# MaxWolf-01/sentinel2-landcover-classification

Measured on AMD Instinct MI355X. Metric: Sentinel-2 256x256x13 tiles/sec fwd+bwd, higher is better.
Workload: dtype f32

## Files before the change

### include/s2k_ops.h

```cpp
#ifndef S2K_OPS_H
#define S2K_OPS_H

#define S2K_N_T 12
#define S2K_N_N 4
#define S2K_N_D 24
#define S2K_N_F 6

#define S2K_BASE_WS 0
#define S2K_BASE_PARAMS 1
#define S2K_BASE_GRADS 2
#define S2K_BASE_BUFS 3
#define S2K_BASE_X 4
#define S2K_BASE_OUT 5
#define S2K_BASE_DOUT 6
#define S2K_BASE_NOISE 7
#define S2K_BASE_WGS 8
#define S2K_BASE_CONST 9
#define S2K_BASE_Y 10
#define S2K_BASE_AUX 11
#define S2K_BASE_WPACK 12
#define S2K_BASE_DX 13
#define S2K_N_BASES 14

#define S2K_PRO_NONE 0
#define S2K_PRO_AFFINE 1
#define S2K_PRO_SILU 2
#define S2K_PRO_RELU 3
#define S2K_PRO_GELU 4
#define S2K_MODE_CONV 0
#define S2K_MODE_CONVT_SCATTER 1
#define S2K_MODE_GATHER2X2 2
#define S2K_FLAG_SIDE 1
#define S2K_FLAG_JOIN 2
#define S2K_FLAG_BF16 4
#define S2K_FLAG_Q4 16
#define S2K_FLAG_DMA 8
#define S2K_FLAG_RES_GELU_GRAD 32
#define S2K_FLAG_SPLIT 64
#define S2K_FLAG_CHAIN 128

#define S2K_OP_MEMSET 1
#define S2K_MEMSET_T_DST 0
#define S2K_MEMSET_N_BYTES 0

#define S2K_OP_AXPY 2
#define S2K_AXPY_T_X 0
#define S2K_AXPY_T_Y 1
#define S2K_AXPY_N_COUNT 0

#define S2K_OP_WEIGHT_PACK 3
#define S2K_WEIGHT_PACK_T_TABLE 0
#define S2K_WEIGHT_PACK_T_SRC 1
#define S2K_WEIGHT_PACK_T_DST 2
#define S2K_WEIGHT_PACK_N_TOTAL 0
#define S2K_WEIGHT_PACK_N_BF16_BASE 1
#define S2K_WEIGHT_PACK_N_Q4_BASE 2
#define S2K_WEIGHT_PACK_N_SPLIT_BASE 3
#define S2K_WEIGHT_PACK_D_N_ENTRIES 0

#define S2K_OP_CONV 4
#define S2K_CONV_T_X1 0
#define S2K_CONV_T_BNV1 1
#define S2K_CONV_T_GATE1 2
#define S2K_CONV_T_X2 3
#define S2K_CONV_T_BNV2 4
#define S2K_CONV_T_WT 5
#define S2K_CONV_T_BIAS 6
#define S2K_CONV_T_Y 7
#define S2K_CONV_T_STATS 8
#define S2K_CONV_T_RES 9
#define S2K_CONV_T_SCRATCH 10
#define S2K_CONV_T_WTB 11
// ... 722 lines not shown
```

### sentinel2-landcover-classification_amd/csrc/dwconv.hip

```cpp
#include <stdlib.h>

#include <algorithm>

#include "common.h"

namespace s2k {

struct DwP {
    const float* x;
    const float* bnv;
    const float* w;
    const float* dy;
    float* out;
    double* stats;
    int B, C, H, W, K, S, PT, PL, HO, WO, pro, beta, nrep;
    int PPB, RT, bands, IRt, LW;
    int XG, LPP, lwp_shift;
    int vps_shift;
    float inv_xg;
    int bloop, cgroups;
    BnFold fold;
};

__device__ __forceinline__ int chan_of(int64_t plane, int C) { return (int)((uint32_t)plane % (uint32_t)C); }
// ... 358 lines not shown
        }
        __builtin_amdgcn_wave_barrier();
#pragma unroll
        for (int g = 0; g < NG; ++g) {
            const int gi = li + 64 * g, r = gi / XGW, xg = gi % XGW;
            float o[4] = {0.f, 0.f, 0.f, 0.f};
            const float* t0 = t + r * TW + 4 * xg;
#pragma unroll
            for (int ky = 0; ky < K; ++ky) {
                float win[12];
                read_window<3>(t0 + ky * TW, win);
#pragma unroll
                for (int kx = 0; kx < K; ++kx)
#pragma unroll
                    for (int j = 0; j < 4; ++j) o[j] = fmaf(wk[ky * K + kx], win[4 - PADK + j + kx], o[j]);
            }
            if (ok) {
                *reinterpret_cast<f32x4*>(p.out + off + 4 * li + 256 * g) = f32x4{o[0], o[1], o[2], o[3]};
#pragma unroll
                for (int j = 0; j < 4; ++j) { s += o[j]; q = fmaf(o[j], o[j], q); }
            }
        }
#pragma unroll
        for (int g = 0; g < NG; ++g) cur[g] = nxt[g];
        hcur = hnxt;
    }
    if (p.stats) {
        const double sd = wave_sum_d((double)s), qd = wave_sum_d((double)q);
        if (lane == 0) {
            double* st = p.stats + (int64_t)((blockIdx.x + blockIdx.y) % p.nrep) * 2 * p.C;
            atomic_add_d(st + c, sd);
            atomic_add_d(st + p.C + c, qd);
        }
    }
}

template <int K, int PRO, int W, int R = W>
__global__ void __launch_bounds__(NTHREADS) dwconv_wgrad_plane_kernel(const DwP p, int bchunk) {
    constexpr int PADK = (K - 1) / 2;
    constexpr bool BAND = R != W;
    constexpr int NB = W / R, GPP = R * W / 4, NG = GPP > 64 ? GPP / 64 : 1, LPP = GPP > 64 ? 64 : GPP, PW = 64 / LPP, XGW = W / 4;
    constexpr int HG = BAND ? (K - 1) * XGW : 0;
    constexpr int TH = R + K - 1, TW = W + 8, TILE = TH * TW, HW = W * W;
    static_assert(HG <= 64 && (!BAND || PW == 1) && W % R == 0, "band geometry");
    extern __shared__ __attribute__((aligned(16))) float smem[];
    const int lane = threadIdx.x & 63, wave = threadIdx.x >> 6;
    const int c = blockIdx.x * 4 + wave;
    if (c >= p.C) return;
    const int n_items = p.B * NB;
    const int i_lo = blockIdx.y * bchunk, i_hi = min(n_items, i_lo + bchunk);
    float sc = 1.0f, sh = 0.0f;
    if (PRO != S2K_PRO_NONE) { sc = p.bnv[c]; sh = p.bnv[p.C + c]; }
    float* tiles = smem + wave * (2 * PW * TILE);
    for (int i = lane; i < 2 * PW * TILE; i += 64) tiles[i] = 0.0f;
    const int sub = lane / LPP, li = lane % LPP;
    const int64_t bstride = (int64_t)p.C * HW, coff = (int64_t)c * HW;
    const f32x4 zero = {0.f, 0.f, 0.f, 0.f};
    const int hrow = lane / XGW, hxg = lane % XGW;
    const int h_trow = hrow < PADK ? hrow : R + hrow;
    const int h_dy = hrow < PADK ? hrow - PADK : R + hrow - PADK;
    auto item_off = [&](int it, int& y0) -> int64_t {
        const int b = BAND ? it / NB : it;
        y0 = BAND ? (it - b * NB) * R : 0;
        return (int64_t)b * bstride + coff + (int64_t)y0 * W;
    };
    f32x4 cur[NG], dcur[NG], hcur = zero;
// ... 1242 lines not shown
    p.dbeta1 = ref_ptr<float>(c, a1.t[S2K_BN_BWD_APPLY_T_DBETA]);
    p.x = ref_ptr<const float>(c, dg.t[S2K_DWCONV_DGRAD_T_XRAW]);
    p.bnv2 = ref_ptr<const float>(c, dg.t[S2K_DWCONV_DGRAD_T_BNV]);
    p.w = ref_ptr<const float>(c, dg.t[S2K_DWCONV_DGRAD_T_WT]);
    p.dw = ref_ptr<float>(c, wg.t[S2K_DWCONV_WGRAD_T_DW]);
    p.g = ref_ptr<float>(c, dg.t[S2K_DWCONV_DGRAD_T_G]);
    p.gamma2 = ref_ptr<const float>(c, a2.t[S2K_BN_BWD_APPLY_T_GAMMA]);
    p.dgamma2 = ref_ptr<float>(c, a2.t[S2K_BN_BWD_APPLY_T_DGAMMA]);
    p.dbeta2 = ref_ptr<float>(c, a2.t[S2K_BN_BWD_APPLY_T_DBETA]);
    const void* all[] = {p.d, p.dy, p.ydw, p.bnv1, p.mulbc, p.addbc, p.ps, p.gamma1, p.dgamma1, p.dbeta1, p.x, p.bnv2, p.w, p.dw, p.g, p.gamma2,
                         p.dgamma2, p.dbeta2};
    for (const void* q : all) {
        if (bad(q)) { set_error("dw_bwd_chain: null base"); return S2K_EFAULT; }
        if (!q) { set_error("dw_bwd_chain: missing tensor"); return S2K_EINVAL; }
    }
    p.B = dg.d[0]; p.C = dg.d[1];
    const int W = dg.d[3], K = dg.d[4];
    p.inv_count1 = 1.0 / (double)a1.n[S2K_BN_BWD_APPLY_N_COUNT];
    p.inv_count2 = 1.0 / (double)a2.n[S2K_BN_BWD_APPLY_N_COUNT];
    p.addscale = a1.f[S2K_BN_BWD_APPLY_F_ADDSCALE];
    const int pw = W == 8 ? 4 : 1;
    const size_t lds = ((size_t)4 * 2 * 2 * pw * (W + K - 1) * (W + 8) + 16 + 4 * K * K) * sizeof(float);
    if (lds > 64 * 1024) { set_error("dw_bwd_chain: tile too large (%zu B)", lds); return S2K_EINVAL; }
    const dim3 grid(p.C);
    if (K == 3 && W == 8) hipLaunchKernelGGL((dw_bwd_chain_kernel<3, 8>), grid, dim3(NTHREADS), lds, c.stream, p);
    else if (K == 3 && W == 16) hipLaunchKernelGGL((dw_bwd_chain_kernel<3, 16>), grid, dim3(NTHREADS), lds, c.stream, p);
    else if (K == 5 && W == 8) hipLaunchKernelGGL((dw_bwd_chain_kernel<5, 8>), grid, dim3(NTHREADS), lds, c.stream, p);
    else if (K == 5 && W == 16) hipLaunchKernelGGL((dw_bwd_chain_kernel<5, 16>), grid, dim3(NTHREADS), lds, c.stream, p);
    else { set_error("dw_bwd_chain: unsupported plane %d, k %d", W, K); return S2K_EINVAL; }
    g_s2k_variant = 10;
    return S2K_OK;
}

}
```

### sentinel2-landcover-classification_amd/csrc/s2k_api.hip

```cpp
#include <cstdarg>
#include <cstdio>
#include <cstring>
#include <mutex>
#include <vector>

#include <stdlib.h>

#include "common.h"

namespace s2k {

static thread_local char g_err[512] = "";
thread_local int g_s2k_variant = 0;

void set_error(const char* fmt, ...) {
    va_list ap;
    va_start(ap, fmt);
    vsnprintf(g_err, sizeof(g_err), fmt, ap);
    va_end(ap);
}

int launch_conv(const S2kOp&, const Ctx&);
int launch_wgrad(const S2kOp&, const Ctx&);
int launch_dwconv_fwd(const S2kOp&, const Ctx&);
// ... 19 lines not shown
int launch_chan_ln_bwd(const S2kOp&, const Ctx&);
int launch_act_bwd(const S2kOp&, const Ctx&);
int launch_act_fwd(const S2kOp&, const Ctx&);
int launch_attn_fwd(const S2kOp&, const Ctx&);
int launch_attn_bwd(const S2kOp&, const Ctx&);
int launch_mae_mask_index(const S2kOp&, const Ctx&);
int launch_token_gather(const S2kOp&, const Ctx&);
int launch_token_scatter(const S2kOp&, const Ctx&);
int launch_patchify(const S2kOp&, const Ctx&);
int launch_mae_loss_fwd(const S2kOp&, const Ctx&);
int launch_mae_loss_bwd(const S2kOp&, const Ctx&);
int launch_transpose_cl(const S2kOp&, const Ctx&);
int launch_drop_gate(const S2kOp&, const Ctx&);
int launch_confusion(const S2kOp&, const Ctx&);
int launch_tile_prep(const S2kOp&, const Ctx&);
int launch_se_bn_sums(const S2kOp&, const Ctx&);
int launch_se_bn_combine(const S2kOp&, const Ctx&);
int launch_space_to_depth(const S2kOp&, const Ctx&);
int launch_se_fc_wgrad(const S2kOp&, const Ctx&);
int launch_ids_to_dec_idx(const S2kOp&, const Ctx&);
int launch_upsample_zero(const S2kOp&, const Ctx&);
int launch_im2col(const S2kOp&, const Ctx&);
int launch_tile_label_hist(const S2kOp&, const Ctx&);
int launch_tile_moments(const S2kOp&, const Ctx&);
int launch_window_blend(const S2kOp&, const Ctx&);
int launch_seg_stats(const S2kOp&, const Ctx&);
int launch_seg_hist(const S2kOp&, const Ctx&);
int launch_grad_clip(const S2kOp&, const Ctx&);
int launch_tile_radix_hist(const S2kOp&, const Ctx&);
int launch_tile_rank_pick(const S2kOp&, const Ctx&);
int launch_tile_quicklook(const S2kOp&, const Ctx&);
int launch_class_overlay(const S2kOp&, const Ctx&);
int launch_dw_bwd_chain(const S2kOp*, const Ctx&);
int launch_adam(float*, const float*, float*, float*, int64_t, double, double, double, double, double, int, hipStream_t);
int launch_mfma_selftest(const float*, const float*, float*, hipStream_t);
int check_mae_panels(const float*, const float*, const float*, const float*, const double*, unsigned char*, float*, int, int, int, int,
                     int, int, int, const int*, int, const int*, int, int, int);
int launch_mae_panels(const float*, const float*, const float*, const float*, const double*, unsigned char*, float*, int, int, int, int,
                      int, int, int, const int*, int, const int*, int, int, int, hipStream_t);
int check_classmap_filter(const void*, int, const int*, void*, int, int, int, int, int, int, int, unsigned, unsigned, int, const unsigned char*,
                          const int*, const int*, int, unsigned long long*, unsigned long long*);
int launch_classmap_filter(const void*, int, const int*, void*, int, int, int, int, int, int, int, unsigned, unsigned, int, const unsigned char*,
                           const int*, const int*, int, unsigned long long*, unsigned long long*, hipStream_t);
int check_classmap_components(const void*, int, const int*, int, int, int, int, int, unsigned, int*, int*, unsigned long long*, unsigned*);
int launch_classmap_components(const void*, int, const int*, int, int, int, int, int, unsigned, int*, int*, unsigned long long*, unsigned*,
                               hipStream_t);
int check_classmap_sieve(const void*, int, const int*, void*, int, int, int, int, int, int, unsigned, int, const int*, const int*,
                         unsigned long long*, const unsigned char*, const int*, const int*, int, unsigned long long*, unsigned long long*,
                         unsigned*);
int launch_classmap_sieve(const void*, int, const int*, void*, int, int, int, int, int, int, unsigned, int, const int*, const int*,
                          unsigned long long*, const unsigned char*, const int*, const int*, int, unsigned long long*, unsigned long long*,
                          unsigned*, hipStream_t);
int check_classmap_distance(const void*, int, const int*, int, int, int, int, int, unsigned, int, unsigned, void*, int*, int*, const void*, int,
                            const int*, int, unsigned long long*);
int launch_classmap_distance(const void*, int, const int*, int, int, int, int, int, unsigned, int, unsigned, void*, int*, int*, const void*, int,
                             const int*, int, unsigned long long*, hipStream_t);
size_t classmap_distance_workspace(int, int, int);
int check_calibration(const float*, int, const void*, int, const int*, int, int, int, unsigned, const float*, int, int, int, float, int, float*,
                      void*, int, unsigned long long*, unsigned long long*, unsigned long long*);
int launch_calibration(const float*, int, const void*, int, const int*, int, int, int, unsigned, const float*, int, int, int, float, int, float*,
                       void*, int, unsigned long long*, unsigned long long*, unsigned long long*, hipStream_t);
int check_rasterize(const int*, int, const int*, const int*, int, const int*, int, const int*, int, int, int, void*, int, int, int, int, void*,
                    long long*, int*);
int launch_rasterize(const int*, int, const int*, const int*, int, const int*, int, const int*, int, int, int, void*, int, int, int, int, void*,
                     long long*, int*, hipStream_t);
size_t rasterize_workspace(int, int);
// ... 172 lines not shown
};

static int try_dw_chain(const S2kOp* ops, int i, int end, const Ctx& c, int* rc) {
    if (!(ops[i].flags & S2K_FLAG_CHAIN) || i + 3 >= end) return 0;
    const S2kOp &a1 = ops[i], &wg = ops[i + 1], &dg = ops[i + 2], &a2 = ops[i + 3];
    if (a1.kind != S2K_OP_BN_BWD_APPLY || wg.kind != S2K_OP_DWCONV_WGRAD || dg.kind != S2K_OP_DWCONV_DGRAD || a2.kind != S2K_OP_BN_BWD_APPLY) return 0;
    if ((a1.flags | wg.flags | dg.flags | a2.flags) & (S2K_FLAG_BF16 | S2K_FLAG_SPLIT)) return 0;
    const int64_t dy = a1.t[S2K_BN_BWD_APPLY_T_DY], x = dg.t[S2K_DWCONV_DGRAD_T_XRAW], g = dg.t[S2K_DWCONV_DGRAD_T_G];
    if (dy < 0 || a1.t[S2K_BN_BWD_APPLY_T_GP] != dy || a1.t[S2K_BN_BWD_APPLY_T_COEF] >= 0 || a1.t[S2K_BN_BWD_APPLY_T_PS] < 0 ||
        a1.t[S2K_BN_BWD_APPLY_T_MULBC] < 0 || a1.t[S2K_BN_BWD_APPLY_T_ADDBC] < 0 || a1.d[S2K_BN_BWD_APPLY_D_ACT] != S2K_PRO_SILU ||
        a1.d[S2K_BN_BWD_APPLY_D_EVAL] || a1.d[S2K_BN_BWD_APPLY_D_OUT_BF16] || a1.n[S2K_BN_BWD_APPLY_N_COUNT] <= 0) return 0;
    if (wg.t[S2K_DWCONV_WGRAD_T_DY] != dy || dg.t[S2K_DWCONV_DGRAD_T_DY] != dy || x < 0 || wg.t[S2K_DWCONV_WGRAD_T_X] != x ||
        dg.t[S2K_DWCONV_DGRAD_T_BNV] < 0 || wg.t[S2K_DWCONV_WGRAD_T_BNV] != dg.t[S2K_DWCONV_DGRAD_T_BNV] || g < 0 || g == dy || g == x ||
        dg.t[S2K_DWCONV_DGRAD_T_STATS2] < 0) return 0;
    for (int k = 0; k <= 10; ++k)
        if (wg.d[k] != dg.d[k]) return 0;
    const int B = dg.d[0], C = dg.d[1], H = dg.d[2], W = dg.d[3], K = dg.d[4];
    if (B <= 0 || C <= 0 || H != W || (W != 8 && W != 16) || (K != 3 && K != 5) || dg.d[5] != 1 || dg.d[6] != (K - 1) / 2 || dg.d[7] != (K - 1) / 2 ||
        dg.d[8] != H || dg.d[9] != W || dg.d[10] != S2K_PRO_SILU || dg.d[S2K_DWCONV_DGRAD_D_BETA] != 0) return 0;
    if ((int64_t)B * C * H * W * 4 >= 0x7ffffff0ll) return 0;
    if (a2.t[S2K_BN_BWD_APPLY_T_GP] != g || a2.t[S2K_BN_BWD_APPLY_T_DY] != g || a2.t[S2K_BN_BWD_APPLY_T_Y] != x ||
        a2.t[S2K_BN_BWD_APPLY_T_BNV] != dg.t[S2K_DWCONV_DGRAD_T_BNV] || a2.t[S2K_BN_BWD_APPLY_T_STATS2] != dg.t[S2K_DWCONV_DGRAD_T_STATS2] ||
        a2.t[S2K_BN_BWD_APPLY_T_COEF] >= 0 || a2.t[S2K_BN_BWD_APPLY_T_PS] >= 0 || a2.t[S2K_BN_BWD_APPLY_T_MULBC] >= 0 ||
        a2.t[S2K_BN_BWD_APPLY_T_ADDBC] >= 0 || a2.d[S2K_BN_BWD_APPLY_D_ACT] != S2K_PRO_NONE || a2.d[S2K_BN_BWD_APPLY_D_EVAL] ||
        a2.d[S2K_BN_BWD_APPLY_D_OUT_BF16] || a2.n[S2K_BN_BWD_APPLY_N_COUNT] <= 0) return 0;
    const int HW = H * W;
    if (a1.d[S2K_BN_BWD_APPLY_D_B] != B || a1.d[S2K_BN_BWD_APPLY_D_C] != C || a1.d[S2K_BN_BWD_APPLY_D_HW] != HW ||
        a2.d[S2K_BN_BWD_APPLY_D_B] != B || a2.d[S2K_BN_BWD_APPLY_D_C] != C || a2.d[S2K_BN_BWD_APPLY_D_HW] != HW) return 0;
    g_s2k_variant = 0;
    *rc = check_launch(launch_dw_bwd_chain(&ops[i], c), ops[i], i);
    return 4;
}

int s2k_program_run(const S2kOp* ops, int begin, int end, void* const* bases, int n_bases, void* stream) {
    if (!ops || !bases || begin < 0 || end < begin) { set_error("program_run: bad arguments"); return S2K_EINVAL; }
    hipStream_t main_st = static_cast<hipStream_t>(stream);
    DeviceGuard guard(main_st);
    Ctx c{bases, n_bases, main_st};
    bool any_side = false;
    for (int i = begin; i < end && !any_side; ++i) any_side = (ops[i].flags & S2K_FLAG_SIDE) != 0;
    SideQueue* sq = any_side ? lease_side_queue(guard.dev) : nullptr;
    bool side_busy = false;
    bool main_dirty = true;
    auto join = [&]() {
        if (!side_busy) return;
        (void)hipEventRecord(sq->join, sq->stream);
        (void)hipStreamWaitEvent(main_st, sq->join, 0);
        side_busy = false;
    };
    int rc = S2K_OK;
    for (int i = begin; i < end; ++i) {
        const S2kOp& op = ops[i];
        if ((op.flags & S2K_FLAG_CHAIN) && i + 3 < end) {
            if ((op.flags | ops[i + 1].flags | ops[i + 2].flags | ops[i + 3].flags) & S2K_FLAG_JOIN) join();
            const int used = try_dw_chain(ops, i, end, c, &rc);
            if (used) {
                main_dirty = true;
                if (rc != S2K_OK) break;
                i += used - 1;
                continue;
            }
        }
        if ((op.flags & S2K_FLAG_SIDE) && sq) {
            if (main_dirty) {
                (void)hipEventRecord(sq->fork, main_st);
                (void)hipStreamWaitEvent(sq->stream, sq->fork, 0);
                main_dirty = false;
            }
            Ctx cs{bases, n_bases, sq->stream};
            rc = check_launch(dispatch(op, cs), op, i);
            side_busy = true;
        } else {
            if (op.flags & S2K_FLAG_JOIN) join();
            rc = check_launch(dispatch(op, c), op, i);
            main_dirty = true;
        }
        if (rc != S2K_OK) break;
    }
    join();
    release_side_queue(guard.dev, sq);
    return rc;
}

int s2k_op_launch(const S2kOp* op, void* const* bases, int n_bases, void* stream) {
    if (!op || !bases) { set_error("op_launch: bad arguments"); return S2K_EINVAL; }
    DeviceGuard guard(static_cast<hipStream_t>(stream));
    Ctx c{bases, n_bases, static_cast<hipStream_t>(stream)};
    return check_launch(dispatch(*op, c), *op, 0);
}

static int profile_impl(const S2kOp* ops, int begin, int end, void* const* bases, int n_bases, void* stream, float* ms_by_kind,
                        int* launches_by_kind, float* ms_per_op, int* variant_per_op);

int s2k_program_profile(const S2kOp* ops, int begin, int end, void* const* bases, int n_bases, void* stream, float* ms_by_kind,
                        int* launches_by_kind) {
// ... 3 lines not shown
int s2k_program_profile_ops(const S2kOp* ops, int begin, int end, void* const* bases, int n_bases, void* stream,
                            float* ms_per_op) {
    float ms[S2K_N_KINDS + 1];
    int cnt[S2K_N_KINDS + 1];
    return profile_impl(ops, begin, end, bases, n_bases, stream, ms, cnt, ms_per_op, nullptr);
}

int s2k_program_profile_variants(const S2kOp* ops, int begin, int end, void* const* bases, int n_bases, void* stream,
                                 float* ms_per_op, int* variant_per_op) {
    float ms[S2K_N_KINDS + 1];
    int cnt[S2K_N_KINDS + 1];
    if (!ms_per_op || !variant_per_op) { set_error("program_profile_variants: bad arguments"); return S2K_EINVAL; }
    return profile_impl(ops, begin, end, bases, n_bases, stream, ms, cnt, ms_per_op, variant_per_op);
}

static int profile_impl(const S2kOp* ops, int begin, int end, void* const* bases, int n_bases, void* stream, float* ms_by_kind,
                        int* launches_by_kind, float* ms_per_op, int* variant_per_op) {
    if (!ops || !bases || !ms_by_kind || !launches_by_kind || begin < 0 || end < begin) {
        set_error("program_profile: bad arguments");
        return S2K_EINVAL;
    }
    hipStream_t st = static_cast<hipStream_t>(stream);
    DeviceGuard guard(st);
    Ctx c{bases, n_bases, st};
    const int n = end - begin;
    hipEvent_t* ev = new hipEvent_t[n + 1];
    for (int i = 0; i <= n; ++i) hipEventCreate(&ev[i]);
    int rc = S2K_OK;
    hipEventRecord(ev[0], st);
    int done = 0;
    std::vector<char> fused(n, 0);
    for (int i = 0; i < n; ++i) {
        g_s2k_variant = 0;
        const int used = try_dw_chain(ops, begin + i, end, c, &rc);
        if (!used) rc = check_launch(dispatch(ops[begin + i], c), ops[begin + i], begin + i);
        if (rc != S2K_OK) break;
        for (int k = 0; k < (used ? used : 1); ++k) {
            if (variant_per_op) variant_per_op[i + k] = g_s2k_variant;
            hipEventRecord(ev[i + k + 1], st);
            if (k) fused[i + k] = 1;
        }
        if (used) i += used - 1;
        done = i + 1;
    }
    hipStreamSynchronize(st);
    if (rc == S2K_OK) {
        for (int k = 0; k <= S2K_N_KINDS; ++k) { ms_by_kind[k] = 0.0f; launches_by_kind[k] = 0; }
        for (int i = 0; i < done; ++i) {
            float ms = 0.0f;
            if (!fused[i]) hipEventElapsedTime(&ms, ev[i], ev[i + 1]);
            const int k = ops[begin + i].kind;
            if (ms_per_op) ms_per_op[i] = ms;
            if (k > 0 && k <= S2K_N_KINDS && !fused[i]) { ms_by_kind[k] += ms; launches_by_kind[k] += 1; }
        }
    }
    for (int i = 0; i <= n; ++i) hipEventDestroy(ev[i]);
    delete[] ev;
    return rc;
}

int s2k_adam_step(float* p, const float* g, float* m, float* v, int64_t n, double lr, double beta1, double beta2, double eps,
                  double weight_decay, int step, void* stream) {
    DeviceGuard guard(static_cast<hipStream_t>(stream));
    const int rc = launch_adam(p, g, m, v, n, lr, beta1, beta2, eps, weight_decay, step, static_cast<hipStream_t>(stream));
    if (rc != S2K_OK) return rc;
    const hipError_t e = hipGetLastError();
    if (e != hipSuccess) { set_error("adam: %s", hipGetErrorString(e)); return S2K_EHIP; }
// ... 123 lines not shown
```

### sentinel2-landcover-classification_amd/plan/opdefs.py

```python
from __future__ import annotations

N_T, N_N, N_D, N_F = 12, 4, 24, 6
OP_BYTES = 8 + 8 * N_T + 8 * N_N + 4 * N_D + 4 * N_F
assert OP_BYTES == 256

BASES = ["WS", "PARAMS", "GRADS", "BUFS", "X", "OUT", "DOUT", "NOISE", "WGS", "CONST", "Y", "AUX", "WPACK", "DX"]
BASE = {n: i for i, n in enumerate(BASES)}

def stats_replicas(C: int) -> int:
    return max(1, min(64, 4096 // max(C, 1)))


PRO_NONE, PRO_AFFINE, PRO_SILU, PRO_RELU, PRO_GELU = 0, 1, 2, 3, 4
ACT_NONE, ACT_SILU, ACT_RELU, ACT_GELU = 0, 2, 3, 4
ACT_MUL = 5
MODE_CONV, MODE_CONVT_SCATTER, MODE_GATHER2X2 = 0, 1, 2
FLAG_SIDE, FLAG_JOIN = 1, 2
FLAG_BF16 = 4
FLAG_Q4 = 16
FLAG_RES_GELU_GRAD = 32
FLAG_SPLIT = 64
FLAG_DMA = 8
FLAG_CHAIN = 128

FOLD_T, FOLD_N, FOLD_D, FOLD_F = ["FSTATS", "FGAMMA", "FBETA", "FRM", "FRV"], ["FCOUNT"], ["FNREP"], ["FEPS", "FMOM"]
FOLD_KINDS = ("DWCONV_FWD", "SE_POOL", "BN_RESIDUAL")

OPS: dict[str, tuple[list[str], list[str], list[str], list[str]]] = {
    "MEMSET": (["DST"], ["BYTES"], [], []),
    "AXPY": (["X", "Y"], ["COUNT"], [], []),
    "WEIGHT_PACK": (["TABLE", "SRC", "DST"], ["TOTAL", "BF16_BASE", "Q4_BASE", "SPLIT_BASE"], ["N_ENTRIES"], []),
    "CONV": (["X1", "BNV1", "GATE1", "X2", "BNV2", "WT", "BIAS", "Y", "STATS", "RES", "SCRATCH", "WTB"], [],
             ["B", "C1", "C2", "H", "W", "M", "KH", "KW", "STRIDE", "PAD_T", "PAD_L", "HO", "WO",
              "PRO1", "PRO2", "MODE", "W_SM", "W_SK", "W_ST", "FLIP", "BETA", "YC", "NREP", "X1_BF16"], []),
    "WGRAD": (["P", "BNVP", "GATEP", "Q", "BNVQ", "GATEQ", "WGS"], [],
              ["B", "M", "C", "CTOT", "H", "W", "KH", "KW", "STRIDE", "PAD_T", "PAD_L", "HO", "WO",
               "PROP", "PROQ", "MODE", "P_BF16"], []),
    "WGRAD_FINALIZE": (["TABLE", "WGS", "GRADS"], ["TOTAL"], ["N_ENTRIES"], []),
    "DWCONV_FWD": (["X", "BNV", "WT", "Y", "STATS"] + FOLD_T, FOLD_N,
                   ["B", "C", "H", "W", "K", "STRIDE", "PAD_T", "PAD_L", "HO", "WO", "PRO", "NREP"] + FOLD_D, FOLD_F),
    "DWCONV_DGRAD": (["DY", "WT", "XRAW", "BNV", "G", "STATS2"], [],
                     ["B", "C", "H", "W", "K", "STRIDE", "PAD_T", "PAD_L", "HO", "WO", "PRO", "BETA", "NREP"], []),
    "DWCONV_WGRAD": (["DY", "X", "BNV", "DW"], [],
                     ["B", "C", "H", "W", "K", "STRIDE", "PAD_T", "PAD_L", "HO", "WO", "PRO"], []),
    "BN_FINALIZE": (["STATS", "GAMMA", "BETA", "RM", "RV", "BNV"], ["COUNT"], ["C", "TRAIN", "NREP"], ["EPS", "MOM"]),
    "SE_POOL": (["Y", "BNV", "POOL"] + FOLD_T, FOLD_N, ["B", "C", "HW", "PRO"] + FOLD_D, FOLD_F),
    "SE_FC": (["POOL", "W1", "B1", "W2", "B2", "HPRE", "GATE"], [], ["B", "C", "CSQ"], []),
    "SE_FC_BWD": (["DGATE", "GATE", "HPRE", "POOL", "W1", "W2", "DW1", "DB1", "DW2", "DB2", "DPOOL", "HS"], [],
                  ["B", "C", "CSQ"], []),
    "SE_BWD_REDUCE": (["G", "Y", "BNV", "DGATE"], [], ["B", "C", "HW", "PRO"], []),
    "BN_BWD_REDUCE": (["G", "Y", "BNV", "MULBC", "ADDBC", "NOISE", "GOUT", "STATS2"], [],
                      ["B", "C", "HW", "ACT", "NREP"], ["KEEP", "ADDSCALE"]),
    "BN_BWD_FINALIZE": (["STATS2", "GAMMA", "BNV", "DGAMMA", "DBETA", "COEF"], ["COUNT"], ["C", "NREP"], []),
    "BN_BWD_APPLY": (["GP", "Y", "BNV", "COEF", "DY", "STATS2", "GAMMA", "DGAMMA", "DBETA", "MULBC", "ADDBC", "PS"], ["COUNT"],
                     ["B", "C", "HW", "NREP", "ACT", "EVAL", "OUT_BF16"], ["ADDSCALE"]),
    "BN_RESIDUAL": (["Y", "BNV", "IDENT", "NOISE", "XOUT"] + FOLD_T, FOLD_N, ["B", "C", "HW"] + FOLD_D, ["KEEP"] + FOLD_F),
# ... 85 lines not shown
```

### sentinel2-landcover-classification_amd/plan/unet_plan.py

```python
from __future__ import annotations

import math
from dataclasses import dataclass, field

from . import opdefs as D
from .program import Arena, Program, TRef

CAT_SIZES = {
    "b0": [592, 296, 152, 80], "b1": [592, 296, 152, 80], "b2": [600, 304, 152, 80],
    "b3": [608, 304, 160, 88], "b4": [624, 312, 160, 88], "b5": [640, 320, 168, 88],
    "b6": [656, 328, 168, 96], "b7": [672, 336, 176, 96],
}


@dataclass
class BlockSpec:
    kernel: int
    stride: int
    cin: int
    cout: int
    expand: int
    se: int
    residual: bool

# ... 879 lines not shown
            continue
        dy, x, g, st2 = a1.get("DY"), dg.get("XRAW"), dg.get("G"), dg.get("STATS2")
        if not (same(a1.get("GP"), dy) and same(wg.get("DY"), dy) and same(dg.get("DY"), dy)
                and same(wg.get("X"), x) and same(a2.get("Y"), x) and same(a2.get("GP"), g) and same(a2.get("DY"), g)
                and same(a2.get("STATS2"), st2) and same(wg.get("BNV"), dg.get("BNV")) and same(a2.get("BNV"), dg.get("BNV"))):
            continue
        if not (a1.get("ACT") == D.ACT_SILU and isinstance(a1.get("PS"), TRef) and isinstance(a1.get("MULBC"), TRef)
                and isinstance(a1.get("ADDBC"), TRef) and a1.get("COEF") is None and not a1.get("EVAL") and not a1.get("OUT_BF16")):
            continue
        if not (a2.get("COEF") is None and not a2.get("ACT") and a2.get("PS") is None and a2.get("MULBC") is None
                and a2.get("ADDBC") is None and not a2.get("EVAL") and not a2.get("OUT_BF16")):
            continue
        geo = ("B", "C", "H", "W", "K", "STRIDE", "PAD_T", "PAD_L", "HO", "WO", "PRO")
        K, W = dg["K"], dg["W"]
        if not (all(wg[k] == dg[k] for k in geo) and dg["STRIDE"] == 1 and dg["PRO"] == D.PRO_SILU and not dg.get("BETA")
                and dg["H"] == W and W in (8, 16) and K in (3, 5) and dg["HO"] == W and dg["WO"] == W
                and dg["PAD_T"] == (K - 1) // 2 and dg["PAD_L"] == (K - 1) // 2):
            continue
        if not all(f["B"] == dg["B"] and f["C"] == dg["C"] and f["HW"] == W * W for f in (a1, a2)):
            continue
        dead = [(t.base, t.off, t.off + t.nbytes) for t in (st2,)]
        live = False
        for _k2, f2 in ops[i + 4:]:
            for v in f2.values():
                if isinstance(v, TRef) and any(v.base == b and v.off < hi and lo < v.off + v.nbytes for (b, lo, hi) in dead):
                    live = True
        if live:
            continue
        a1["_flags"] = a1.get("_flags", 0) | D.FLAG_CHAIN
        marked += 1
    return marked


def fold_bn_finalize(prog: Program) -> int:
    if tune("S2K_FOLD_BN", "1") != "1":
        return 0
    ops = prog.ops
    folded = 0
    i = 0
    while i < len(ops):
        kind, f = ops[i]
        if kind != "BN_FINALIZE" or not f.get("TRAIN") or f.get("_flags"):
            i += 1
            continue
        bnv = f["BNV"]
        touched = {t.ref for k in ("BNV", "RM", "RV", "STATS") if isinstance(t := f.get(k), TRef)}
        target = None
        for j in range(i + 1, len(ops)):
            k2, f2 = ops[j]
            refs = {v.ref for v in f2.values() if isinstance(v, TRef)}
            if not (refs & touched):
                continue
            if (k2 in D.FOLD_KINDS and isinstance(f2.get("BNV"), TRef) and f2["BNV"].ref == bnv.ref and f2.get("FSTATS") is None
                    and f2.get("C") == f["C"] and f2.get("PRO", 1) and len(refs & touched) == 1 and not f2.get("_flags")):
                target = j
            break
        if target is None:
            i += 1
            continue
        ops[target][1].update(FSTATS=f["STATS"], FGAMMA=f["GAMMA"], FBETA=f["BETA"], FRM=f["RM"], FRV=f["RV"], FCOUNT=f["COUNT"],
                              FNREP=f["NREP"], FEPS=f["EPS"], FMOM=f["MOM"])
        del ops[i]
        folded += 1
    return folded


# ... 66 lines not shown
        raise ValueError(f"EfficientnetUnet needs H, W multiples of 32, got {H}x{W}")
    layout = layout or build_layout(spec)
    p = _P(spec, layout, B, H, W, training, want_bwd)
    p.defer_wgrads = defer_wgrads
    p.bf16 = bool(bf16)
    p.split = bool(split)
    eps, mom = spec.bn_eps, spec.bn_momentum
    x_in = Act(TRef(D.BASE["X"], 0, (B, spec.in_channels, H, W), "f32", "x"), spec.in_channels, H, W,
               needs_grad=bool(want_dx), grad=TRef(D.BASE["DX"], 0, (B, spec.in_channels, H, W), "f32", "dx") if want_dx else None)

    cur, fmaps, _ = emit_encoder(p, spec, x_in, "encoder.")

    ups_out = [512, 256, 128, 64]
    cat = CAT_SIZES[spec.version]
    for i, fm in enumerate(fmaps):
        u = conv_transpose(p, f"up_convs.{i}.weight", f"up_convs.{i}.bias", cur, ups_out[i])
        if u.C + fm.C != cat[i] or (u.H, u.W) != (fm.H, fm.W):
            raise ValueError(f"decoder level {i}: cat {u.C}+{fm.C} != {cat[i]} or size mismatch")
        pre = f"double_convs.{i}"
        a = conv_bn(p, pre + ".0.weight", pre + ".1", [u, fm], ups_out[i], 3, 1, False, D.PRO_RELU, 1e-5, 0.1,
                    bias=pre + ".0.bias")
        cur = conv_bn(p, pre + ".3.weight", pre + ".4", [a], ups_out[i], 3, 1, False, D.PRO_RELU, 1e-5, 0.1,
                      bias=pre + ".3.bias")
    u = conv_transpose(p, "input_up_conv.weight", "input_up_conv.bias", cur, 32)
    pre = "input_double_conv"
    a = conv_bn(p, pre + ".0.weight", pre + ".1", [u, x_in], 32, 3, 1, False, D.PRO_RELU, 1e-5, 0.1,
                bias=pre + ".0.bias")
    cur = conv_bn(p, pre + ".3.weight", pre + ".4", [a], 32, 3, 1, False, D.PRO_RELU, 1e-5, 0.1,
                  bias=pre + ".3.bias")
    logits = out_conv(p, "out_conv1x1.weight", "out_conv1x1.bias", cur, spec.num_classes)

    segments, bwd = finish_plan(p, layout, training, bucket_floats)
    fold_bn_finalize(p.fwd)

    return UnetPlan(spec, B, H, W, training, p.fwd, bwd, p.ws.mark(), p.aux.mark(), p.blob, layout, len(spec.blocks),
                    segments if p.want_bwd else [], (B, spec.num_classes, H, W), p.tensors, p.wpack.mark())
```

Baseline: 1008.

## Fuse depthwise conv forward with SE pool on small planes

Adds a fused kernel that runs the depthwise conv forward for one channel across the whole batch in a single block. It keeps the conv outputs in LDS, reduces the BN statistics inside the block, folds the BN finalize, and computes the SE average pool from LDS. This removes a separate SE_POOL launch, the re-read of the conv output, and the cross-block atomic statistics. In exchange each channel runs as a single block, which limits parallelism, and the LDS needed grows with batch size; if it exceeds 64KB the code falls back to the unfused ops. The planner marks eligible pairs by default through a tune flag.

```diff
diff --git a/include/s2k_ops.h b/include/s2k_ops.h
--- a/include/s2k_ops.h
+++ b/include/s2k_ops.h
@@ -38,6 +38,7 @@
 #define S2K_FLAG_RES_GELU_GRAD 32
 #define S2K_FLAG_SPLIT 64
 #define S2K_FLAG_CHAIN 128
+#define S2K_FLAG_FWD_CHAIN 256
 
 #define S2K_OP_MEMSET 1
 #define S2K_MEMSET_T_DST 0
diff --git a/sentinel2-landcover-classification_amd/csrc/dwconv.hip b/sentinel2-landcover-classification_amd/csrc/dwconv.hip
--- a/sentinel2-landcover-classification_amd/csrc/dwconv.hip
+++ b/sentinel2-landcover-classification_amd/csrc/dwconv.hip
@@ -414,6 +414,100 @@
             atomic_add_d(st + c, sd);
             atomic_add_d(st + p.C + c, qd);
         }
+    }
+}
+
+template <int K, int W>
+__global__ void __launch_bounds__(NTHREADS) dw_fwd_pool_kernel(const DwP p, const BnFold pf, float* pool) {
+    constexpr int PADK = (K - 1) / 2, KK = K * K;
+    constexpr int GPP = W * W / 4, LPP = GPP > 64 ? 64 : GPP, PW = 64 / LPP, XGW = W / 4;
+    constexpr int TH = W + K - 1, TW = W + 8, TILE = TH * TW, HW = W * W;
+    constexpr int WAVE_TILES = 2 * PW * TILE;
+    static_assert(GPP == 64 || GPP == 16, "8 x 8 or 16 x 16 planes");
+    static_assert(WAVE_TILES % 4 == 0, "the output planes behind the tiles stay 16-byte aligned");
+    extern __shared__ __attribute__((aligned(16))) float smem[];
+    const int lane = threadIdx.x & 63, wave = threadIdx.x >> 6;
+    const int c = blockIdx.x;
+    const int B = p.B, C = p.C;
+    const int sub = lane / LPP, li = lane % LPP;
+    const int r = li / XGW, xg = li % XGW;
+    const int64_t bstride = (int64_t)C * HW;
+    const int64_t loff = (int64_t)c * HW + 4 * li;
+    const f32x4 zero = {0.f, 0.f, 0.f, 0.f};
+    const int b_first = wave * PW + sub;
+    f32x4 cur = *reinterpret_cast<const f32x4*>(p.x + (int64_t)min(b_first, B - 1) * bstride + loff);
+    float sc, sh;
+    if (p.fold.stats) bn_fold_wave(p.fold, C, c, wave == 0, sc, sh);
+    else { sc = p.bnv[c]; sh = p.bnv[C + c]; }
+    float wk[KK];
+#pragma unroll
+    for (int i = 0; i < KK; ++i) wk[i] = p.w[c * KK + i];
+    float* tiles = smem + wave * WAVE_TILES;
+    for (int i = lane; i < WAVE_TILES / 4; i += 64) reinterpret_cast<f32x4*>(tiles)[i] = zero;
+    float* ybuf = smem + 4 * WAVE_TILES;
+    double* red = reinterpret_cast<double*>(ybuf + (int64_t)B * HW);
+    float s = 0.0f, q = 0.0f;
+    int buf = 0;
+    for (int b = b_first; b - sub < B; b += 4 * PW, buf ^= 1) {
+        const bool ok = b < B;
+        const f32x4 nxt = *reinterpret_cast<const f32x4*>(p.x + (int64_t)min(b + 4 * PW, B - 1) * bstride + loff);
+        f32x4 v;
+#pragma unroll
+        for (int j = 0; j < 4; ++j) v[j] = apply_pro_c<S2K_PRO_SILU>(cur[j], sc, sh);
+        if (!ok) v = zero;
+        float* t = tiles + (buf * PW + sub) * TILE;
+        *reinterpret_cast<f32x4*>(t + (r + PADK) * TW + 4 + 4 * xg) = v;
+        __builtin_amdgcn_wave_barrier();
+        float o[4] = {0.f, 0.f, 0.f, 0.f};
+        const float* t0 = t + r * TW + 4 * xg;
+#pragma unroll
+        for (int ky = 0; ky < K; ++ky) {
+            float win[12];
+            read_window<3>(t0 + ky * TW, win);
+#pragma unroll
+            for (int kx = 0; kx < K; ++kx)
+#pragma unroll
+                for (int j = 0; j < 4; ++j) o[j] = fmaf(wk[ky * K + kx], win[4 - PADK + j + kx], o[j]);
+        }
+        if (ok) {
+            const f32x4 ov = {o[0], o[1], o[2], o[3]};
+            *reinterpret_cast<f32x4*>(p.out + (int64_t)b * bstride + loff) = ov;
+            *reinterpret_cast<f32x4*>(ybuf + b * HW + 4 * li) = ov;
+#pragma unroll
+            for (int j = 0; j < 4; ++j) { s += o[j]; q = fmaf(o[j], o[j], q); }
+        }
+        cur = nxt;
+    }
+    {
+        const double sd = wave_sum_d((double)s), qd = wave_sum_d((double)q);
+        if (lane == 0) { red[wave * 2] = sd; red[wave * 2 + 1] = qd; }
+        if (wave == 0) {
+            double s0 = 0.0, q0 = 0.0;
+            for (int rp = lane; rp < pf.nrep; rp += 64) { s0 += pf.stats[(int64_t)rp * 2 * C + c]; q0 += pf.stats[(int64_t)rp * 2 * C + C + c]; }
+            s0 = wave_sum_d(s0);
+            q0 = wave_sum_d(q0);
+            if (lane == 0) { red[8] = s0; red[9] = q0; }
+        }
+    }
+    __syncthreads();
+    const double t1 = (red[0] + red[2]) + (red[4] + red[6]), t2 = (red[1] + red[3]) + (red[5] + red[7]);
+    float scale, shift;
+    bn_fold_finish(pf, C, c, red[8] + t1, red[9] + t2, threadIdx.x == 0, scale, shift);
+    if (threadIdx.x == 0) {
+        p.stats[c] += t1;
+        p.stats[C + c] += t2;
+    }
+    const float inv = 1.0f / (float)HW;
+    for (int b = b_first; b - sub < B; b += 4 * PW) {
+        float sp = 0.0f;
+        if (b < B) {
+            const f32x4 v = *reinterpret_cast<const f32x4*>(ybuf + b * HW + 4 * li);
+            const float a0 = apply_pro(v[0], S2K_PRO_SILU, scale, shift), a1 = apply_pro(v[1], S2K_PRO_SILU, scale, shift);
+            const float a2 = apply_pro(v[2], S2K_PRO_SILU, scale, shift), a3 = apply_pro(v[3], S2K_PRO_SILU, scale, shift);
+            sp = (a0 + a1) + (a2 + a3);
+        }
+        sp = group_sum(sp, LPP);
+        if (li == 0 && b < B) pool[(int64_t)b * C + c] = sp * inv;
     }
 }
 
@@ -1722,4 +1816,39 @@
     return S2K_OK;
 }
 
-}
+int launch_dw_fwd_pool(const S2kOp* o, const Ctx& c) {
+    const S2kOp &dw = o[0], &sp = o[1];
+    DwP p{};
+    if (int e = fill_geo(p, dw.d)) return e;
+    p.x = ref_ptr<const float>(c, dw.t[S2K_DWCONV_FWD_T_X]);
+    p.bnv = ref_ptr<const float>(c, dw.t[S2K_DWCONV_FWD_T_BNV]);
+    p.w = ref_ptr<const float>(c, dw.t[S2K_DWCONV_FWD_T_WT]);
+    p.out = ref_ptr<float>(c, dw.t[S2K_DWCONV_FWD_T_Y]);
+    p.stats = ref_ptr<double>(c, dw.t[S2K_DWCONV_FWD_T_STATS]);
+    float* bnv2 = ref_ptr<float>(c, sp.t[S2K_SE_POOL_T_BNV]);
+    float* pool = ref_ptr<float>(c, sp.t[S2K_SE_POOL_T_POOL]);
+    const void* all[] = {p.x, p.bnv, p.w, p.out, p.stats, bnv2, pool};
+    for (const void* q : all) {
+        if (bad(q)) { set_error("dw_fwd_pool: null base"); return S2K_EFAULT; }
+        if (!q) { set_error("dw_fwd_pool: missing tensor"); return S2K_EINVAL; }
+    }
+    if (int e = fill_bn_fold(p.fold, c, &dw.t[S2K_DWCONV_FWD_T_FSTATS], dw.n[S2K_DWCONV_FWD_N_FCOUNT], dw.d[S2K_DWCONV_FWD_D_FNREP],
+                             dw.f[S2K_DWCONV_FWD_F_FEPS], dw.f[S2K_DWCONV_FWD_F_FMOM], const_cast<float*>(p.bnv), "dw_fwd_pool")) return e;
+    BnFold pf;
+    if (int e = fill_bn_fold(pf, c, &sp.t[S2K_SE_POOL_T_FSTATS], sp.n[S2K_SE_POOL_N_FCOUNT], sp.d[S2K_SE_POOL_D_FNREP], sp.f[S2K_SE_POOL_F_FEPS],
+                             sp.f[S2K_SE_POOL_F_FMOM], bnv2, "dw_fwd_pool")) return e;
+    if (!pf.stats || p.pro != S2K_PRO_SILU) { set_error("dw_fwd_pool: needs SiLU prologues and the pool's folded BN_FINALIZE"); return S2K_EINVAL; }
+    const int pw = p.W == 8 ? 4 : 1;
+    const size_t lds = ((size_t)4 * 2 * pw * (p.W + p.K - 1) * (p.W + 8) + (size_t)p.B * p.H * p.W) * sizeof(float) + 10 * sizeof(double);
+    if (lds > 64 * 1024) return 1;
+    const dim3 grid(p.C);
+    if (p.K == 3 && p.W == 8) hipLaunchKernelGGL((dw_fwd_pool_kernel<3, 8>), grid, dim3(NTHREADS), lds, c.stream, p, pf, pool);
+    else if (p.K == 3 && p.W == 16) hipLaunchKernelGGL((dw_fwd_pool_kernel<3, 16>), grid, dim3(NTHREADS), lds, c.stream, p, pf, pool);
+    else if (p.K == 5 && p.W == 8) hipLaunchKernelGGL((dw_fwd_pool_kernel<5, 8>), grid, dim3(NTHREADS), lds, c.stream, p, pf, pool);
+    else if (p.K == 5 && p.W == 16) hipLaunchKernelGGL((dw_fwd_pool_kernel<5, 16>), grid, dim3(NTHREADS), lds, c.stream, p, pf, pool);
+    else { set_error("dw_fwd_pool: unsupported plane %d, k %d", p.W, p.K); return S2K_EINVAL; }
+    g_s2k_variant = 16;
+    return S2K_OK;
+}
+
+}
diff --git a/sentinel2-landcover-classification_amd/csrc/s2k_api.hip b/sentinel2-landcover-classification_amd/csrc/s2k_api.hip
--- a/sentinel2-landcover-classification_amd/csrc/s2k_api.hip
+++ b/sentinel2-landcover-classification_amd/csrc/s2k_api.hip
@@ -75,6 +75,7 @@
 int launch_tile_quicklook(const S2kOp&, const Ctx&);
 int launch_class_overlay(const S2kOp&, const Ctx&);
 int launch_dw_bwd_chain(const S2kOp*, const Ctx&);
+int launch_dw_fwd_pool(const S2kOp*, const Ctx&);
 int launch_adam(float*, const float*, float*, float*, int64_t, double, double, double, double, double, int, hipStream_t);
 int launch_mfma_selftest(const float*, const float*, float*, hipStream_t);
 int check_mae_panels(const float*, const float*, const float*, const float*, const double*, unsigned char*, float*, int, int, int, int,
@@ -313,6 +314,36 @@
     return 4;
 }
 
+static int try_dw_fwd_pool(const S2kOp* ops, int i, int end, const Ctx& c, int* rc) {
+    if (!(ops[i].flags & S2K_FLAG_FWD_CHAIN) || i + 1 >= end) return 0;
+    const S2kOp &dw = ops[i], &sp = ops[i + 1];
+    if (dw.kind != S2K_OP_DWCONV_FWD || sp.kind != S2K_OP_SE_POOL) return 0;
+    if ((dw.flags | sp.flags) & (S2K_FLAG_SIDE | S2K_FLAG_BF16 | S2K_FLAG_SPLIT)) return 0;
+    const int64_t y = dw.t[S2K_DWCONV_FWD_T_Y], st = dw.t[S2K_DWCONV_FWD_T_STATS];
+    if (y < 0 || st < 0 || dw.t[S2K_DWCONV_FWD_T_X] < 0 || dw.t[S2K_DWCONV_FWD_T_BNV] < 0 || dw.t[S2K_DWCONV_FWD_T_WT] < 0 ||
+        sp.t[S2K_SE_POOL_T_Y] != y || sp.t[S2K_SE_POOL_T_FSTATS] != st || sp.t[S2K_SE_POOL_T_BNV] < 0 || sp.t[S2K_SE_POOL_T_POOL] < 0) return 0;
+    for (int k = S2K_SE_POOL_T_FGAMMA; k <= S2K_SE_POOL_T_FRV; ++k)
+        if (sp.t[k] < 0) return 0;
+    const int B = dw.d[S2K_DWCONV_FWD_D_B], C = dw.d[S2K_DWCONV_FWD_D_C], H = dw.d[S2K_DWCONV_FWD_D_H], W = dw.d[S2K_DWCONV_FWD_D_W];
+    const int K = dw.d[S2K_DWCONV_FWD_D_K], nrep = dw.d[S2K_DWCONV_FWD_D_NREP] > 0 ? dw.d[S2K_DWCONV_FWD_D_NREP] : 1;
+    if (B <= 0 || C <= 0 || H != W || (W != 8 && W != 16) || (K != 3 && K != 5) || dw.d[S2K_DWCONV_FWD_D_STRIDE] != 1 ||
+        dw.d[S2K_DWCONV_FWD_D_PAD_T] != (K - 1) / 2 || dw.d[S2K_DWCONV_FWD_D_PAD_L] != (K - 1) / 2 || dw.d[S2K_DWCONV_FWD_D_HO] != H ||
+        dw.d[S2K_DWCONV_FWD_D_WO] != W || dw.d[S2K_DWCONV_FWD_D_PRO] != S2K_PRO_SILU) return 0;
+    if ((int64_t)B * C * H * W * 4 >= 0x7ffffff0ll) return 0;
+    if (sp.d[S2K_SE_POOL_D_B] != B || sp.d[S2K_SE_POOL_D_C] != C || sp.d[S2K_SE_POOL_D_HW] != H * W || sp.d[S2K_SE_POOL_D_PRO] != S2K_PRO_SILU ||
+        (sp.d[S2K_SE_POOL_D_FNREP] > 0 ? sp.d[S2K_SE_POOL_D_FNREP] : 1) != nrep || sp.n[S2K_SE_POOL_N_FCOUNT] != (int64_t)B * H * W) return 0;
+    if (dw.t[S2K_DWCONV_FWD_T_FSTATS] >= 0) {
+        for (int k = S2K_DWCONV_FWD_T_FGAMMA; k <= S2K_DWCONV_FWD_T_FRV; ++k)
+            if (dw.t[k] < 0) return 0;
+        if (dw.n[S2K_DWCONV_FWD_N_FCOUNT] <= 0) return 0;
+    }
+    g_s2k_variant = 0;
+    const int lrc = launch_dw_fwd_pool(&ops[i], c);
+    if (lrc == 1) return 0;
+    *rc = check_launch(lrc, ops[i], i);
+    return 2;
+}
+
 int s2k_program_run(const S2kOp* ops, int begin, int end, void* const* bases, int n_bases, void* stream) {
     if (!ops || !bases || begin < 0 || end < begin) { set_error("program_run: bad arguments"); return S2K_EINVAL; }
     hipStream_t main_st = static_cast<hipStream_t>(stream);
@@ -342,6 +373,16 @@
                 continue;
             }
         }
+        if ((op.flags & S2K_FLAG_FWD_CHAIN) && i + 1 < end) {
+            if ((op.flags | ops[i + 1].flags) & S2K_FLAG_JOIN) join();
+            const int used = try_dw_fwd_pool(ops, i, end, c, &rc);
+            if (used) {
+                main_dirty = true;
+                if (rc != S2K_OK) break;
+                i += used - 1;
+                continue;
+            }
+        }
         if ((op.flags & S2K_FLAG_SIDE) && sq) {
             if (main_dirty) {
                 (void)hipEventRecord(sq->fork, main_st);
@@ -411,7 +452,8 @@
     std::vector<char> fused(n, 0);
     for (int i = 0; i < n; ++i) {
         g_s2k_variant = 0;
-        const int used = try_dw_chain(ops, begin + i, end, c, &rc);
+        int used = try_dw_chain(ops, begin + i, end, c, &rc);
+        if (!used) used = try_dw_fwd_pool(ops, begin + i, end, c, &rc);
         if (!used) rc = check_launch(dispatch(ops[begin + i], c), ops[begin + i], begin + i);
         if (rc != S2K_OK) break;
         for (int k = 0; k < (used ? used : 1); ++k) {
diff --git a/sentinel2-landcover-classification_amd/plan/opdefs.py b/sentinel2-landcover-classification_amd/plan/opdefs.py
--- a/sentinel2-landcover-classification_amd/plan/opdefs.py
+++ b/sentinel2-landcover-classification_amd/plan/opdefs.py
@@ -22,6 +22,7 @@
 FLAG_SPLIT = 64
 FLAG_DMA = 8
 FLAG_CHAIN = 128
+FLAG_FWD_CHAIN = 256
 
 FOLD_T, FOLD_N, FOLD_D, FOLD_F = ["FSTATS", "FGAMMA", "FBETA", "FRM", "FRV"], ["FCOUNT"], ["FNREP"], ["FEPS", "FMOM"]
 FOLD_KINDS = ("DWCONV_FWD", "SE_POOL", "BN_RESIDUAL")
diff --git a/sentinel2-landcover-classification_amd/plan/unet_plan.py b/sentinel2-landcover-classification_amd/plan/unet_plan.py
--- a/sentinel2-landcover-classification_amd/plan/unet_plan.py
+++ b/sentinel2-landcover-classification_amd/plan/unet_plan.py
@@ -935,6 +935,33 @@
     return marked
 
 
+def mark_dw_fwd_chain(prog: Program) -> int:
+    if tune("S2K_DW_FWD_CHAIN", "1") != "1":
+        return 0
+    ops = prog.ops
+
+    def same(a, b):
+        return isinstance(a, TRef) and isinstance(b, TRef) and a.ref == b.ref
+
+    marked = 0
+    for i in range(len(ops) - 1):
+        (k1, dw), (k2, sp) = ops[i], ops[i + 1]
+        if (k1, k2) != ("DWCONV_FWD", "SE_POOL") or dw.get("_flags", 0) or sp.get("_flags", 0):
+            continue
+        K, W = dw["K"], dw["W"]
+        if not (same(sp.get("Y"), dw.get("Y")) and same(sp.get("FSTATS"), dw.get("STATS")) and isinstance(dw.get("BNV"), TRef)
+                and isinstance(sp.get("BNV"), TRef) and sp.get("FNREP") == dw.get("NREP")
+                and sp.get("FCOUNT") == dw["B"] * dw["HO"] * dw["WO"]):
+            continue
+        if not (dw["PRO"] == D.PRO_SILU and sp["PRO"] == D.PRO_SILU and dw["STRIDE"] == 1 and dw["H"] == W and W in (8, 16) and K in (3, 5)
+                and dw["HO"] == W and dw["WO"] == W and dw["PAD_T"] == (K - 1) // 2 and dw["PAD_L"] == (K - 1) // 2
+                and sp["B"] == dw["B"] and sp["C"] == dw["C"] and sp["HW"] == W * W):
+            continue
+        dw["_flags"] = dw.get("_flags", 0) | D.FLAG_FWD_CHAIN
+        marked += 1
+    return marked
+
+
 def fold_bn_finalize(prog: Program) -> int:
     if tune("S2K_FOLD_BN", "1") != "1":
         return 0
@@ -1067,6 +1094,7 @@
 
     segments, bwd = finish_plan(p, layout, training, bucket_floats)
     fold_bn_finalize(p.fwd)
+    mark_dw_fwd_chain(p.fwd)
 
     return UnetPlan(spec, B, H, W, training, p.fwd, bwd, p.ws.mark(), p.aux.mark(), p.blob, layout, len(spec.blocks),
                     segments if p.want_bwd else [], (B, spec.num_classes, H, W), p.tensors, p.wpack.mark())
```

Result: no change. 1013 (median of 6 runs) (+0.5%).
